# paultsw/wavenet-speech

Hardware: AMD Instinct MI355X
Metric: samples/sec fwd+bwd, 256-ch 30-block WaveNet @16k seq (higher is better)
Workload: dtype f32; 1 GPU; BASELINE.json configs[2]: WaveNet 256 ch, 30 blocks (3 x dilation 1..512), k=2, seq_len 16000, batch 16 per GPU, f32, full step (fwd+bwd+grad all-reduce+Adam); channels=256, blocks=30, seq_len=16000, batch_per_gpu=16, global_batch=16, parallelism=dp1, params=16037632, input=dense one-hot, init=reference

## Files before the change

wavenet_speech_amd/csrc/wn_gemm.hip:

```cpp
#include <cstdlib>
#include <type_traits>

#include "wn_kernels.h"
#include "wn_knobs.h"

namespace wn {

__device__ __forceinline__ int rowof(int r, int h) { return (r & 3) + 8 * (r >> 2) + 4 * h; }

__device__ __forceinline__ float sigmoid_f(float x) {
    const float e = __builtin_amdgcn_exp2f(-1.44269504088896341f * x);
    return __builtin_amdgcn_rcpf(1.0f + e);
}
__device__ __forceinline__ float tanh_f(float x) {
    const float ax = __builtin_fabsf(x);
    const float e = __builtin_amdgcn_exp2f(-2.88539008177792681f * ax);
    const float big = (1.0f - e) * __builtin_amdgcn_rcpf(1.0f + e);
    const float x2 = x * x;
    const float small = ax * (1.0f + x2 * (-0.333333333f + x2 * (0.133333333f + x2 * -0.0539682540f)));
    return __builtin_copysignf(ax < 0.125f ? small : big, x);
}

template <int NT> struct BVec;
template <> struct BVec<4> { typedef f32x4 reg_t; };
template <> struct BVec<2> { typedef float __attribute__((ext_vector_type(2))) reg_t; };

template <int MT, int NT, int EPI, int PFB, int WPS>
__global__ __launch_bounds__(64, WPS) void series_gemm_kernel(const GemmArgs a) {
    typedef typename BVec<NT>::reg_t breg_t;
    constexpr int COLS = 32 * NT;
    const int lane = threadIdx.x;
    const int n0 = lane & 31, h0 = lane >> 5;
#ifdef WN_STAMPS
    const unsigned long long st_t0 = __builtin_amdgcn_s_memtime(), st_r0 = __builtin_amdgcn_s_memrealtime();
    unsigned long long st_t1 = 0, st_t2 = 0;
#endif

    const int id = blockIdx.x;
    const int xcd = id & 7, local = id >> 3;
    const int slab_i = local % a.nslab;
    const int coltile = (local / a.nslab) * 8 + xcd;
    if (coltile >= a.ncol) return;
    const int b = coltile / a.tiles_per_row;
    const int t0 = (coltile - b * a.tiles_per_row) * COLS;
    const GemmSlab sl = a.slab[slab_i];
    const int ld = a.ld;

    f32x16 acc[MT][NT];
    const float* bias_p = (a.bias ? a.bias : a.wpacked) + sl.boff;
    const float bias_on = a.bias ? 1.0f : 0.0f;
#pragma unroll
    for (int m = 0; m < MT; ++m) {
#pragma unroll
        for (int r = 0; r < 16; ++r) {
            const float bv = bias_p[32 * m + rowof(r, h0)] * bias_on;
#pragma unroll
            for (int t = 0; t < NT; ++t) acc[m][t][r] = bv;
        }
    }

    int nkb = 0;
    for (int s = 0; s < sl.nseg; ++s) nkb += a.seg[s].nkb;

    constexpr unsigned kRsrcFlags = 0x00020000u;
    auto resource = [&](const float* base) {
        return __builtin_amdgcn_make_buffer_rsrc(const_cast<float*>(base), 0, 0xffffffffu, kRsrcFlags);
    };
    const __amdgpu_buffer_rsrc_t wrs = resource(a.wpacked + sl.woff);
    const unsigned a_off = lane * 16u;
    unsigned a_soff = 0;
    const long tilebase = (long)a.halo + t0;
    unsigned b_off[4];
#pragma unroll
    for (int q = 0; q < 4; ++q) b_off[q] = 4u * ((unsigned)(4 * h0 + q) * (unsigned)ld + (unsigned)(NT * n0));
    int seg = 0;
    int seg_left = a.seg[0].nkb;
    __amdgpu_buffer_rsrc_t brs = resource(a.seg[0].base + (long)b * a.seg[0].cp * ld);
    unsigned b_soff = 4u * (unsigned)(tilebase + a.seg[0].off);
    int b_left = nkb;
    const unsigned a_last = (unsigned)(nkb > 0 ? nkb - 1 : 0) * (MT * 1024u);

    f32x4 A[2][MT];
    breg_t B[4][4];
    auto loadA = [&](f32x4 (&dst)[MT]) {
#pragma unroll
        for (int m = 0; m < MT; ++m)
            dst[m] = __builtin_bit_cast(f32x4, __builtin_amdgcn_raw_buffer_load_b128(wrs, a_off + m * 1024u, a_soff, 0));
        a_soff = min(a_soff + MT * 1024u, a_last);
    };
    auto loadB = [&](breg_t (&dst)[4]) {
#pragma unroll
        for (int q = 0; q < 4; ++q) {
            if constexpr (NT == 4) dst[q] = __builtin_bit_cast(breg_t, __builtin_amdgcn_raw_buffer_load_b128(brs, b_off[q], b_soff, 0));
            else dst[q] = __builtin_bit_cast(breg_t, __builtin_amdgcn_raw_buffer_load_b64(brs, b_off[q], b_soff, 0));
        }
        const int more = min(b_left - 1, 1);
        b_left -= more;
        b_soff += (unsigned)more * (32u * (unsigned)ld);
        seg_left -= more;
        if (b_left > 1 - more && seg_left == 0) {
            ++seg;
            const GemmSeg ns = a.seg[seg];
            seg_left = ns.nkb;
            brs = resource(ns.base + (long)b * ns.cp * ld);
            b_soff = 4u * (unsigned)(tilebase + ns.off);
        }
    };
    auto compute = [&](const f32x4 (&fa)[MT], const breg_t (&fb)[4]) {
#pragma unroll
        for (int q = 0; q < 4; ++q)
#pragma unroll
            for (int m = 0; m < MT; ++m)
#pragma unroll
                for (int t = 0; t < NT; ++t)
                    acc[m][t] = __builtin_amdgcn_mfma_f32_32x32x2f32(fa[m][q], fb[q][t], acc[m][t], 0, 0, 0);
    };

    loadA(A[0]);
#pragma unroll
    for (int p = 0; p < PFB; ++p) loadB(B[p]);
#ifdef WN_STAMPS
    __builtin_amdgcn_sched_barrier(0);
    st_t1 = __builtin_amdgcn_s_memtime();
    __builtin_amdgcn_sched_barrier(0);
#endif
    int g0 = 0;
    for (; g0 + 4 <= nkb; g0 += 4) {
#pragma unroll
        for (int j = 0; j < 4; ++j) {
            loadA(A[(j + 1) & 1]);
            loadB(B[(j + PFB) & 3]);
            __builtin_amdgcn_sched_barrier(0);
            compute(A[j & 1], B[j & 3]);
            __builtin_amdgcn_sched_barrier(0);
        }
    }
#pragma unroll
    for (int j = 0; j < 3; ++j) {
        if (g0 + j < nkb) {
            loadA(A[(j + 1) & 1]);
            loadB(B[(j + PFB) & 3]);
            __builtin_amdgcn_sched_barrier(0);
            compute(A[j & 1], B[j & 3]);
            __builtin_amdgcn_sched_barrier(0);
        }
    }

#ifdef WN_STAMPS
    __builtin_amdgcn_sched_barrier(0);
    st_t2 = __builtin_amdgcn_s_memtime();
    __builtin_amdgcn_sched_barrier(0);
    struct StampOut {
        unsigned long long* p; unsigned long long t0, r0, t1, t2; int lane;
        __device__ ~StampOut() {
            __builtin_amdgcn_sched_barrier(0);
            const unsigned long long t_issued = __builtin_amdgcn_s_memtime();
            __builtin_amdgcn_sched_barrier(0);
            asm volatile("s_waitcnt vmcnt(0)" ::: "memory");
            if (p && lane == 0) {
                p[0] = t0; p[1] = t1; p[2] = t2; p[3] = __builtin_amdgcn_s_memtime();
                p[4] = r0; p[5] = __builtin_amdgcn_s_memrealtime();
                p[6] = __builtin_amdgcn_s_getreg(63492);
                p[7] = (unsigned long long)__builtin_amdgcn_s_getreg(63508) | ((t_issued - t2) << 32);
            }
        }
    } stamp_out{a.stamps ? a.stamps + 8ull * blockIdx.x : nullptr, st_t0, st_r0, st_t1, st_t2, lane};
#endif
    const int lane_e = (int)__builtin_amdgcn_mbcnt_hi(~0u, __builtin_amdgcn_mbcnt_lo(~0u, 0u));
    const int n = lane_e & 31, h = lane_e >> 5;
    const long colbase = tilebase + NT * n;
    const int c0 = t0 + NT * n;
    if (c0 >= a.L) return;
    auto clip = [&](breg_t v) {
#pragma unroll
        for (int t = 1; t < NT; ++t)
            if (c0 + t >= a.L) v[t] = 0.0f;
        return v;
    };
    [[maybe_unused]] auto both_forms = [&](int rows, auto&& body) {
        if (sl.row0 + 32 * MT <= rows && t0 + COLS <= a.L) body(std::true_type{});
        else body(std::false_type{});
    };

    if constexpr (EPI == EPI_LINEAR) {
        const GemmDst d = a.dst[sl.dst];
#pragma unroll
        for (int m = 0; m < MT; ++m) {
#pragma unroll
            for (int r = 0; r < 16; ++r) {
                const int row = sl.row0 + 32 * m + rowof(r, h);
                if (row < d.rows) {
                    float* p = d.base + ((long)b * d.cp + row) * ld + colbase;
                    breg_t v;
#pragma unroll
                    for (int t = 0; t < NT; ++t) v[t] = acc[m][t][r];
                    *reinterpret_cast<breg_t*>(p) = clip(v);
                }
            }
            __builtin_amdgcn_sched_barrier(0);
        }
    } else if constexpr (EPI == EPI_ACCUM) {
        const GemmDst d = a.dst[sl.dst];
        constexpr int RB = 8, BPT = 16 / RB, NBATCH = MT * BPT;
        float* const tile = d.base + (long)b * d.cp * ld + colbase;
        both_forms(d.rows, [&](auto full) {
            constexpr bool FULL = decltype(full)::value;
            breg_t old[2][RB];
            auto fetch = [&](int bi, breg_t (&dst)[RB]) {
                const int m = bi / BPT, r0 = (bi % BPT) * RB;
#pragma unroll
                for (int i = 0; i < RB; ++i) {
                    int row = sl.row0 + 32 * m + rowof(r0 + i, h);
                    if constexpr (!FULL) row = row < d.rows ? row : d.rows - 1;
                    dst[i] = *reinterpret_cast<const breg_t*>(tile + (long)row * ld);
                }
            };
            fetch(0, old[0]);
#pragma unroll
            for (int bi = 0; bi < NBATCH; ++bi) {
                if (bi + 1 < NBATCH) fetch(bi + 1, old[(bi + 1) & 1]);
                __builtin_amdgcn_sched_barrier(0);
                const int m = bi / BPT, r0 = (bi % BPT) * RB;
#pragma unroll
                for (int i = 0; i < RB; ++i) {
                    const int row = sl.row0 + 32 * m + rowof(r0 + i, h);
                    if (FULL || row < d.rows) {
                        breg_t v;
#pragma unroll
                        for (int t = 0; t < NT; ++t) v[t] = acc[m][t][r0 + i] + old[bi & 1][i][t];
                        *reinterpret_cast<breg_t*>(tile + (long)row * ld) = FULL ? v : clip(v);
                    }
                }
                __builtin_amdgcn_sched_barrier(0);
            }
        });
    } else if constexpr (EPI == EPI_GATE) {
#pragma unroll
        for (int i = 0; i < MT / 2; ++i) {
#pragma unroll
            for (int r = 0; r < 16; ++r) {
                const int ch = sl.row0 + 32 * i + rowof(r, h);
                if (ch < a.gate_rows) {
                    breg_t vs, vz;
#pragma unroll
                    for (int t = 0; t < NT; ++t) {
                        const float tt = tanh_f(acc[2 * i][t][r]);
                        const float ss = sigmoid_f(acc[2 * i + 1][t][r]);
                        vs[t] = ss;
                        vz[t] = tt * ss;
                    }
                    const long o = ((long)b * a.gate_cp + ch) * ld + colbase;
                    *reinterpret_cast<breg_t*>(a.z + o) = clip(vz);
                    if (a.sg) *reinterpret_cast<breg_t*>(a.sg + o) = clip(vs);
                }
            }
            __builtin_amdgcn_sched_barrier(0);
        }
    } else if constexpr (EPI == EPI_LEAKY) {
        const GemmDst d = a.dst[sl.dst];
        const float slope = a.slope;
#pragma unroll
        for (int m = 0; m < MT; ++m) {
#pragma unroll
            for (int r = 0; r < 16; ++r) {
                const int row = sl.row0 + 32 * m + rowof(r, h);
                if (row < d.rows) {
                    float* p = d.base + ((long)b * d.cp + row) * ld + colbase;
                    breg_t v;
#pragma unroll
                    for (int t = 0; t < NT; ++t) {
                        const float x = acc[m][t][r];
                        v[t] = x > 0.0f ? x : x * slope;
                    }
                    *reinterpret_cast<breg_t*>(p) = clip(v);
                }
            }
            __builtin_amdgcn_sched_barrier(0);
        }
    } else if constexpr (EPI == EPI_DMASK) {
        const GemmDst d = a.dst[sl.dst];
        const float slope = a.slope;
        constexpr int RB = 8, BPT = 16 / RB, NBATCH = MT * BPT;
        const long tile_off = (long)b * d.cp * ld + colbase;
        float* const tile = d.base + tile_off;
        const float* const mtile = a.mask + tile_off;
        both_forms(d.rows, [&](auto full) {
            constexpr bool FULL = decltype(full)::value;
            breg_t msk[2][RB];
            auto fetch = [&](int bi, breg_t (&dst)[RB]) {
                const int m = bi / BPT, r0 = (bi % BPT) * RB;
#pragma unroll
                for (int i = 0; i < RB; ++i) {
                    int row = sl.row0 + 32 * m + rowof(r0 + i, h);
                    if constexpr (!FULL) row = row < d.rows ? row : d.rows - 1;
                    dst[i] = *reinterpret_cast<const breg_t*>(mtile + (long)row * ld);
                }
            };
            fetch(0, msk[0]);
#pragma unroll
            for (int bi = 0; bi < NBATCH; ++bi) {
                if (bi + 1 < NBATCH) fetch(bi + 1, msk[(bi + 1) & 1]);
                __builtin_amdgcn_sched_barrier(0);
                const int m = bi / BPT, r0 = (bi % BPT) * RB;
#pragma unroll
                for (int i = 0; i < RB; ++i) {
                    const int row = sl.row0 + 32 * m + rowof(r0 + i, h);
                    if (FULL || row < d.rows) {
                        breg_t v;
#pragma unroll
                        for (int t = 0; t < NT; ++t) {
                            const float g = acc[m][t][r0 + i];
                            v[t] = msk[bi & 1][i][t] > 0.0f ? g : g * slope;
                        }
                        *reinterpret_cast<breg_t*>(tile + (long)row * ld) = FULL ? v : clip(v);
                    }
                }
                __builtin_amdgcn_sched_barrier(0);
            }
        });
    } else {
        constexpr int RB = (MT == 4) ? 8 : 4;
        constexpr int BPT = 16 / RB;
        constexpr int NBATCH = MT * BPT;
        both_forms(a.gate_rows, [&](auto full) {
            constexpr bool FULL = decltype(full)::value;
            breg_t vt[2][RB], vs[2][RB];
            const long plane = (long)b * a.gate_cp * ld;
            auto at = [&](auto* base, int ch) {
                if constexpr (FULL) return (decltype(base))((char*)(base + plane) + 4u * ((unsigned)ch * (unsigned)ld + (unsigned)colbase));
                else return base + ((long)b * a.gate_cp + ch) * ld + colbase;
            };
            auto fetch = [&](int bi, breg_t (&ft)[RB], breg_t (&fs)[RB]) {
                const int m = bi / BPT, r0 = (bi % BPT) * RB;
#pragma unroll
                for (int i = 0; i < RB; ++i) {
                    int ch = sl.row0 + 32 * m + rowof(r0 + i, h);
                    if constexpr (!FULL) ch = ch < a.gate_rows ? ch : a.gate_rows - 1;
                    ft[i] = *reinterpret_cast<const breg_t*>(at(a.z, ch));
                    fs[i] = *reinterpret_cast<const breg_t*>(at(a.sg, ch));
                }
            };
            fetch(0, vt[0], vs[0]);
#pragma unroll
            for (int bi = 0; bi < NBATCH; ++bi) {
                if (bi + 1 < NBATCH) fetch(bi + 1, vt[(bi + 1) & 1], vs[(bi + 1) & 1]);
                __builtin_amdgcn_sched_barrier(0);
                const int m = bi / BPT, r0 = (bi % BPT) * RB;
#pragma unroll
                for (int i = 0; i < RB; ++i) {
                    const int r = r0 + i;
                    const int ch = sl.row0 + 32 * m + rowof(r, h);
                    if (FULL || ch < a.gate_rows) {
                        const breg_t z_ = vt[bi & 1][i], sg_ = vs[bi & 1][i];
                        breg_t va, vg;
#pragma unroll
                        for (int t = 0; t < NT; ++t) {
                            const float dz = acc[m][t][r];
                            const float tt = sg_[t] > 0.0f ? z_[t] / sg_[t] : 0.0f;
                            va[t] = dz * (sg_[t] - z_[t] * tt);
                            vg[t] = dz * z_[t] * (1.0f - sg_[t]);
                        }
                        *reinterpret_cast<breg_t*>(at(a.da, ch)) = FULL ? va : clip(va);
                        *reinterpret_cast<breg_t*>(at(a.dg, ch)) = FULL ? vg : clip(vg);
                    }
                }
                __builtin_amdgcn_sched_barrier(0);
            }
        });
    }
}

#ifdef WN_STAMPS
static unsigned long long* g_stamp_buf = nullptr;
static int g_stamp_kc = -1;
int g_debug_kc = -1;
extern "C" void wn_debug_set_stamp_buffer(void* p) { g_stamp_buf = (unsigned long long*)p; }
extern "C" void wn_debug_set_stamp_class(int kc) { g_stamp_kc = kc; }
extern "C" unsigned wn_debug_last_grid = 0;
#endif

template <int MT, int NT, int EPI, int PFB, int WPS>
static hipError_t launch_one(GemmArgs a, hipStream_t st) {
#ifdef WN_STAMPS
    const bool stamp_this = g_stamp_buf && (g_stamp_kc < 0 || g_stamp_kc == g_debug_kc);
    a.stamps = stamp_this ? g_stamp_buf : nullptr;
#endif
    a.tiles_per_row = (a.L + 32 * NT - 1) / (32 * NT);
    a.ncol = a.B * a.tiles_per_row;
    const int ncol8 = (a.ncol + 7) / 8 * 8;
    const unsigned grid = (unsigned)(a.nslab * ncol8);
#ifdef WN_STAMPS
    if (stamp_this) wn_debug_last_grid = grid;
#endif
    hipLaunchKernelGGL((series_gemm_kernel<MT, NT, EPI, PFB, WPS>), dim3(grid), dim3(64), 0, st, a);
    return hipGetLastError();
}

template <int EPI>
static hipError_t launch_epi(int MT, const GemmArgs& a, hipStream_t st) {
    if (MT == 4) {
        if constexpr (kMeasureBuild) {
            if (measure_knob(Knob::WN_GEMM_VARIANT, 0) == 1) return launch_one<4, 4, EPI, 1, 1>(a, st);
        }
        return launch_one<4, 4, EPI, 3, 1>(a, st);
    }
    if (MT == 2) return launch_one<2, 4, EPI, 3, 2>(a, st);
    if constexpr (EPI != EPI_GATE) {
        if (MT == 1) return launch_one<1, 4, EPI, 3, 2>(a, st);
    }
    return hipErrorInvalidValue;
}

hipError_t launch_gemm(int MT, int epi, const GemmArgs& a, hipStream_t st) {
    if (a.nslab <= 0 || a.B <= 0 || a.L <= 0) return hipSuccess;
    switch (epi) {
        case EPI_LINEAR: return launch_epi<EPI_LINEAR>(MT, a, st);
        case EPI_GATE: return launch_epi<EPI_GATE>(MT, a, st);
        case EPI_DGATE: return launch_epi<EPI_DGATE>(MT, a, st);
        case EPI_ACCUM: return launch_epi<EPI_ACCUM>(MT, a, st);
        case EPI_LEAKY: return launch_epi<EPI_LEAKY>(MT, a, st);
        case EPI_DMASK: return launch_epi<EPI_DMASK>(MT, a, st);
    }
    return hipErrorInvalidValue;
}

}
```

Before: 101.5 samples/s.

## Add finishing-wave path that overlaps last k-blocks with epilogue for linear/leaky GEMMs

```diff
diff --git a/wavenet_speech_amd/csrc/wn_gemm.hip b/wavenet_speech_amd/csrc/wn_gemm.hip
--- a/wavenet_speech_amd/csrc/wn_gemm.hip
+++ b/wavenet_speech_amd/csrc/wn_gemm.hip
@@ -25,349 +25,37 @@
 template <> struct BVec<4> { typedef f32x4 reg_t; };
 template <> struct BVec<2> { typedef float __attribute__((ext_vector_type(2))) reg_t; };
 
+typedef unsigned u32x4 __attribute__((ext_vector_type(4)));
+
+#ifndef WN_FINISH_LINEAR
+#define WN_FINISH_LINEAR 2
+#endif
+constexpr int finish_blocks(int MT, int NT, int EPI, int PFB, int WPS) {
+    return (MT == 4 && NT == 4 && PFB == 3 && WPS == 1 && (EPI == EPI_LINEAR || EPI == EPI_LEAKY)) ? WN_FINISH_LINEAR : 0;
+}
+
+template <int MT, int NT, int EPI, int PFB, int WPS, int FT>
+__device__ __forceinline__ void series_gemm_finishing_wave(const GemmArgs& a) {
+#include "wn_gemm_wave.h"
+}
+
 template <int MT, int NT, int EPI, int PFB, int WPS>
 __global__ __launch_bounds__(64, WPS) void series_gemm_kernel(const GemmArgs a) {
-    typedef typename BVec<NT>::reg_t breg_t;
-    constexpr int COLS = 32 * NT;
-    const int lane = threadIdx.x;
-    const int n0 = lane & 31, h0 = lane >> 5;
-#ifdef WN_STAMPS
-    const unsigned long long st_t0 = __builtin_amdgcn_s_memtime(), st_r0 = __builtin_amdgcn_s_memrealtime();
-    unsigned long long st_t1 = 0, st_t2 = 0;
-#endif
-
-    const int id = blockIdx.x;
-    const int xcd = id & 7, local = id >> 3;
-    const int slab_i = local % a.nslab;
-    const int coltile = (local / a.nslab) * 8 + xcd;
-    if (coltile >= a.ncol) return;
-    const int b = coltile / a.tiles_per_row;
-    const int t0 = (coltile - b * a.tiles_per_row) * COLS;
-    const GemmSlab sl = a.slab[slab_i];
-    const int ld = a.ld;
-
-    f32x16 acc[MT][NT];
-    const float* bias_p = (a.bias ? a.bias : a.wpacked) + sl.boff;
-    const float bias_on = a.bias ? 1.0f : 0.0f;
-#pragma unroll
-    for (int m = 0; m < MT; ++m) {
-#pragma unroll
-        for (int r = 0; r < 16; ++r) {
-            const float bv = bias_p[32 * m + rowof(r, h0)] * bias_on;
-#pragma unroll
-            for (int t = 0; t < NT; ++t) acc[m][t][r] = bv;
+    if constexpr (finish_blocks(MT, NT, EPI, PFB, WPS) > 0) {
+        constexpr int FIN = finish_blocks(MT, NT, EPI, PFB, WPS);
+        const int local = blockIdx.x >> 3;
+        const int coltile = (local / a.nslab) * 8 + (blockIdx.x & 7);
+        const GemmSlab sl = a.slab[local % a.nslab];
+        int nkb = 0;
+        for (int s = 0; s < sl.nseg; ++s) nkb += a.seg[s].nkb;
+        const int t0 = (coltile % a.tiles_per_row) * 32 * NT;
+        if (coltile < a.ncol && nkb >= FIN && sl.row0 + 32 * MT <= a.dst[sl.dst].rows && t0 + 32 * NT <= a.L) {
+            series_gemm_finishing_wave<MT, NT, EPI, PFB, WPS, FIN>(a);
+            return;
         }
     }
-
-    int nkb = 0;
-    for (int s = 0; s < sl.nseg; ++s) nkb += a.seg[s].nkb;
-
-    constexpr unsigned kRsrcFlags = 0x00020000u;
-    auto resource = [&](const float* base) {
-        return __builtin_amdgcn_make_buffer_rsrc(const_cast<float*>(base), 0, 0xffffffffu, kRsrcFlags);
-    };
-    const __amdgpu_buffer_rsrc_t wrs = resource(a.wpacked + sl.woff);
-    const unsigned a_off = lane * 16u;
-    unsigned a_soff = 0;
-    const long tilebase = (long)a.halo + t0;
-    unsigned b_off[4];
-#pragma unroll
-    for (int q = 0; q < 4; ++q) b_off[q] = 4u * ((unsigned)(4 * h0 + q) * (unsigned)ld + (unsigned)(NT * n0));
-    int seg = 0;
-    int seg_left = a.seg[0].nkb;
-    __amdgpu_buffer_rsrc_t brs = resource(a.seg[0].base + (long)b * a.seg[0].cp * ld);
-    unsigned b_soff = 4u * (unsigned)(tilebase + a.seg[0].off);
-    int b_left = nkb;
-    const unsigned a_last = (unsigned)(nkb > 0 ? nkb - 1 : 0) * (MT * 1024u);
-
-    f32x4 A[2][MT];
-    breg_t B[4][4];
-    auto loadA = [&](f32x4 (&dst)[MT]) {
-#pragma unroll
-        for (int m = 0; m < MT; ++m)
-            dst[m] = __builtin_bit_cast(f32x4, __builtin_amdgcn_raw_buffer_load_b128(wrs, a_off + m * 1024u, a_soff, 0));
-        a_soff = min(a_soff + MT * 1024u, a_last);
-    };
-    auto loadB = [&](breg_t (&dst)[4]) {
-#pragma unroll
-        for (int q = 0; q < 4; ++q) {
-            if constexpr (NT == 4) dst[q] = __builtin_bit_cast(breg_t, __builtin_amdgcn_raw_buffer_load_b128(brs, b_off[q], b_soff, 0));
-            else dst[q] = __builtin_bit_cast(breg_t, __builtin_amdgcn_raw_buffer_load_b64(brs, b_off[q], b_soff, 0));
-        }
-        const int more = min(b_left - 1, 1);
-        b_left -= more;
-        b_soff += (unsigned)more * (32u * (unsigned)ld);
-        seg_left -= more;
-        if (b_left > 1 - more && seg_left == 0) {
-            ++seg;
-            const GemmSeg ns = a.seg[seg];
-            seg_left = ns.nkb;
-            brs = resource(ns.base + (long)b * ns.cp * ld);
-            b_soff = 4u * (unsigned)(tilebase + ns.off);
-        }
-    };
-    auto compute = [&](const f32x4 (&fa)[MT], const breg_t (&fb)[4]) {
-#pragma unroll
-        for (int q = 0; q < 4; ++q)
-#pragma unroll
-            for (int m = 0; m < MT; ++m)
-#pragma unroll
-                for (int t = 0; t < NT; ++t)
-                    acc[m][t] = __builtin_amdgcn_mfma_f32_32x32x2f32(fa[m][q], fb[q][t], acc[m][t], 0, 0, 0);
-    };
-
-    loadA(A[0]);
-#pragma unroll
-    for (int p = 0; p < PFB; ++p) loadB(B[p]);
-#ifdef WN_STAMPS
-    __builtin_amdgcn_sched_barrier(0);
-    st_t1 = __builtin_amdgcn_s_memtime();
-    __builtin_amdgcn_sched_barrier(0);
-#endif
-    int g0 = 0;
-    for (; g0 + 4 <= nkb; g0 += 4) {
-#pragma unroll
-        for (int j = 0; j < 4; ++j) {
-            loadA(A[(j + 1) & 1]);
-            loadB(B[(j + PFB) & 3]);
-            __builtin_amdgcn_sched_barrier(0);
-            compute(A[j & 1], B[j & 3]);
-            __builtin_amdgcn_sched_barrier(0);
-        }
-    }
-#pragma unroll
-    for (int j = 0; j < 3; ++j) {
-        if (g0 + j < nkb) {
-            loadA(A[(j + 1) & 1]);
-            loadB(B[(j + PFB) & 3]);
-            __builtin_amdgcn_sched_barrier(0);
-            compute(A[j & 1], B[j & 3]);
-            __builtin_amdgcn_sched_barrier(0);
-        }
-    }
-
-#ifdef WN_STAMPS
-    __builtin_amdgcn_sched_barrier(0);
-    st_t2 = __builtin_amdgcn_s_memtime();
-    __builtin_amdgcn_sched_barrier(0);
-    struct StampOut {
-        unsigned long long* p; unsigned long long t0, r0, t1, t2; int lane;
-        __device__ ~StampOut() {
-            __builtin_amdgcn_sched_barrier(0);
-            const unsigned long long t_issued = __builtin_amdgcn_s_memtime();
-            __builtin_amdgcn_sched_barrier(0);
-            asm volatile("s_waitcnt vmcnt(0)" ::: "memory");
-            if (p && lane == 0) {
-                p[0] = t0; p[1] = t1; p[2] = t2; p[3] = __builtin_amdgcn_s_memtime();
-                p[4] = r0; p[5] = __builtin_amdgcn_s_memrealtime();
-                p[6] = __builtin_amdgcn_s_getreg(63492);
-                p[7] = (unsigned long long)__builtin_amdgcn_s_getreg(63508) | ((t_issued - t2) << 32);
-            }
-        }
-    } stamp_out{a.stamps ? a.stamps + 8ull * blockIdx.x : nullptr, st_t0, st_r0, st_t1, st_t2, lane};
-#endif
-    const int lane_e = (int)__builtin_amdgcn_mbcnt_hi(~0u, __builtin_amdgcn_mbcnt_lo(~0u, 0u));
-    const int n = lane_e & 31, h = lane_e >> 5;
-    const long colbase = tilebase + NT * n;
-    const int c0 = t0 + NT * n;
-    if (c0 >= a.L) return;
-    auto clip = [&](breg_t v) {
-#pragma unroll
-        for (int t = 1; t < NT; ++t)
-            if (c0 + t >= a.L) v[t] = 0.0f;
-        return v;
-    };
-    [[maybe_unused]] auto both_forms = [&](int rows, auto&& body) {
-        if (sl.row0 + 32 * MT <= rows && t0 + COLS <= a.L) body(std::true_type{});
-        else body(std::false_type{});
-    };
-
-    if constexpr (EPI == EPI_LINEAR) {
-        const GemmDst d = a.dst[sl.dst];
-#pragma unroll
-        for (int m = 0; m < MT; ++m) {
-#pragma unroll
-            for (int r = 0; r < 16; ++r) {
-                const int row = sl.row0 + 32 * m + rowof(r, h);
-                if (row < d.rows) {
-                    float* p = d.base + ((long)b * d.cp + row) * ld + colbase;
-                    breg_t v;
-#pragma unroll
-                    for (int t = 0; t < NT; ++t) v[t] = acc[m][t][r];
-                    *reinterpret_cast<breg_t*>(p) = clip(v);
-                }
-            }
-            __builtin_amdgcn_sched_barrier(0);
-        }
-    } else if constexpr (EPI == EPI_ACCUM) {
-        const GemmDst d = a.dst[sl.dst];
-        constexpr int RB = 8, BPT = 16 / RB, NBATCH = MT * BPT;
-        float* const tile = d.base + (long)b * d.cp * ld + colbase;
-        both_forms(d.rows, [&](auto full) {
-            constexpr bool FULL = decltype(full)::value;
-            breg_t old[2][RB];
-            auto fetch = [&](int bi, breg_t (&dst)[RB]) {
-                const int m = bi / BPT, r0 = (bi % BPT) * RB;
-#pragma unroll
-                for (int i = 0; i < RB; ++i) {
-                    int row = sl.row0 + 32 * m + rowof(r0 + i, h);
-                    if constexpr (!FULL) row = row < d.rows ? row : d.rows - 1;
-                    dst[i] = *reinterpret_cast<const breg_t*>(tile + (long)row * ld);
-                }
-            };
-            fetch(0, old[0]);
-#pragma unroll
-            for (int bi = 0; bi < NBATCH; ++bi) {
-                if (bi + 1 < NBATCH) fetch(bi + 1, old[(bi + 1) & 1]);
-                __builtin_amdgcn_sched_barrier(0);
-                const int m = bi / BPT, r0 = (bi % BPT) * RB;
-#pragma unroll
-                for (int i = 0; i < RB; ++i) {
-                    const int row = sl.row0 + 32 * m + rowof(r0 + i, h);
-                    if (FULL || row < d.rows) {
-                        breg_t v;
-#pragma unroll
-                        for (int t = 0; t < NT; ++t) v[t] = acc[m][t][r0 + i] + old[bi & 1][i][t];
-                        *reinterpret_cast<breg_t*>(tile + (long)row * ld) = FULL ? v : clip(v);
-                    }
-                }
-                __builtin_amdgcn_sched_barrier(0);
-            }
-        });
-    } else if constexpr (EPI == EPI_GATE) {
-#pragma unroll
-        for (int i = 0; i < MT / 2; ++i) {
-#pragma unroll
-            for (int r = 0; r < 16; ++r) {
-                const int ch = sl.row0 + 32 * i + rowof(r, h);
-                if (ch < a.gate_rows) {
-                    breg_t vs, vz;
-#pragma unroll
-                    for (int t = 0; t < NT; ++t) {
-                        const float tt = tanh_f(acc[2 * i][t][r]);
-                        const float ss = sigmoid_f(acc[2 * i + 1][t][r]);
-                        vs[t] = ss;
-                        vz[t] = tt * ss;
-                    }
-                    const long o = ((long)b * a.gate_cp + ch) * ld + colbase;
-                    *reinterpret_cast<breg_t*>(a.z + o) = clip(vz);
-                    if (a.sg) *reinterpret_cast<breg_t*>(a.sg + o) = clip(vs);
-                }
-            }
-            __builtin_amdgcn_sched_barrier(0);
-        }
-    } else if constexpr (EPI == EPI_LEAKY) {
-        const GemmDst d = a.dst[sl.dst];
-        const float slope = a.slope;
-#pragma unroll
-        for (int m = 0; m < MT; ++m) {
-#pragma unroll
-            for (int r = 0; r < 16; ++r) {
-                const int row = sl.row0 + 32 * m + rowof(r, h);
-                if (row < d.rows) {
-                    float* p = d.base + ((long)b * d.cp + row) * ld + colbase;
-                    breg_t v;
-#pragma unroll
-                    for (int t = 0; t < NT; ++t) {
-                        const float x = acc[m][t][r];
-                        v[t] = x > 0.0f ? x : x * slope;
-                    }
-                    *reinterpret_cast<breg_t*>(p) = clip(v);
-                }
-            }
-            __builtin_amdgcn_sched_barrier(0);
-        }
-    } else if constexpr (EPI == EPI_DMASK) {
-        const GemmDst d = a.dst[sl.dst];
-        const float slope = a.slope;
-        constexpr int RB = 8, BPT = 16 / RB, NBATCH = MT * BPT;
-        const long tile_off = (long)b * d.cp * ld + colbase;
-        float* const tile = d.base + tile_off;
-        const float* const mtile = a.mask + tile_off;
-        both_forms(d.rows, [&](auto full) {
-            constexpr bool FULL = decltype(full)::value;
-            breg_t msk[2][RB];
-            auto fetch = [&](int bi, breg_t (&dst)[RB]) {
-                const int m = bi / BPT, r0 = (bi % BPT) * RB;
-#pragma unroll
-                for (int i = 0; i < RB; ++i) {
-                    int row = sl.row0 + 32 * m + rowof(r0 + i, h);
-                    if constexpr (!FULL) row = row < d.rows ? row : d.rows - 1;
-                    dst[i] = *reinterpret_cast<const breg_t*>(mtile + (long)row * ld);
-                }
-            };
-            fetch(0, msk[0]);
-#pragma unroll
-            for (int bi = 0; bi < NBATCH; ++bi) {
-                if (bi + 1 < NBATCH) fetch(bi + 1, msk[(bi + 1) & 1]);
-                __builtin_amdgcn_sched_barrier(0);
-                const int m = bi / BPT, r0 = (bi % BPT) * RB;
-#pragma unroll
-                for (int i = 0; i < RB; ++i) {
-                    const int row = sl.row0 + 32 * m + rowof(r0 + i, h);
-                    if (FULL || row < d.rows) {
-                        breg_t v;
-#pragma unroll
-                        for (int t = 0; t < NT; ++t) {
-                            const float g = acc[m][t][r0 + i];
-                            v[t] = msk[bi & 1][i][t] > 0.0f ? g : g * slope;
-                        }
-                        *reinterpret_cast<breg_t*>(tile + (long)row * ld) = FULL ? v : clip(v);
-                    }
-                }
-                __builtin_amdgcn_sched_barrier(0);
-            }
-        });
-    } else {
-        constexpr int RB = (MT == 4) ? 8 : 4;
-        constexpr int BPT = 16 / RB;
-        constexpr int NBATCH = MT * BPT;
-        both_forms(a.gate_rows, [&](auto full) {
-            constexpr bool FULL = decltype(full)::value;
-            breg_t vt[2][RB], vs[2][RB];
-            const long plane = (long)b * a.gate_cp * ld;
-            auto at = [&](auto* base, int ch) {
-                if constexpr (FULL) return (decltype(base))((char*)(base + plane) + 4u * ((unsigned)ch * (unsigned)ld + (unsigned)colbase));
-                else return base + ((long)b * a.gate_cp + ch) * ld + colbase;
-            };
-            auto fetch = [&](int bi, breg_t (&ft)[RB], breg_t (&fs)[RB]) {
-                const int m = bi / BPT, r0 = (bi % BPT) * RB;
-#pragma unroll
-                for (int i = 0; i < RB; ++i) {
-                    int ch = sl.row0 + 32 * m + rowof(r0 + i, h);
-                    if constexpr (!FULL) ch = ch < a.gate_rows ? ch : a.gate_rows - 1;
-                    ft[i] = *reinterpret_cast<const breg_t*>(at(a.z, ch));
-                    fs[i] = *reinterpret_cast<const breg_t*>(at(a.sg, ch));
-                }
-            };
-            fetch(0, vt[0], vs[0]);
-#pragma unroll
-            for (int bi = 0; bi < NBATCH; ++bi) {
-                if (bi + 1 < NBATCH) fetch(bi + 1, vt[(bi + 1) & 1], vs[(bi + 1) & 1]);
-                __builtin_amdgcn_sched_barrier(0);
-                const int m = bi / BPT, r0 = (bi % BPT) * RB;
-#pragma unroll
-                for (int i = 0; i < RB; ++i) {
-                    const int r = r0 + i;
-                    const int ch = sl.row0 + 32 * m + rowof(r, h);
-                    if (FULL || ch < a.gate_rows) {
-                        const breg_t z_ = vt[bi & 1][i], sg_ = vs[bi & 1][i];
-                        breg_t va, vg;
-#pragma unroll
-                        for (int t = 0; t < NT; ++t) {
-                            const float dz = acc[m][t][r];
-                            const float tt = sg_[t] > 0.0f ? z_[t] / sg_[t] : 0.0f;
-                            va[t] = dz * (sg_[t] - z_[t] * tt);
-                            vg[t] = dz * z_[t] * (1.0f - sg_[t]);
-                        }
-                        *reinterpret_cast<breg_t*>(at(a.da, ch)) = FULL ? va : clip(va);
-                        *reinterpret_cast<breg_t*>(at(a.dg, ch)) = FULL ? vg : clip(vg);
-                    }
-                }
-                __builtin_amdgcn_sched_barrier(0);
-            }
-        });
-    }
+    constexpr int FT = 0;
+#include "wn_gemm_wave.h"
 }
 
 #ifdef WN_STAMPS
diff --git a/wavenet_speech_amd/csrc/wn_gemm_wave.h b/wavenet_speech_amd/csrc/wn_gemm_wave.h
--- /dev/null
+++ b/wavenet_speech_amd/csrc/wn_gemm_wave.h
@@ -0,0 +1,407 @@
+    typedef typename BVec<NT>::reg_t breg_t;
+    constexpr int COLS = 32 * NT;
+    const int lane = threadIdx.x;
+    const int n0 = lane & 31, h0 = lane >> 5;
+#ifdef WN_STAMPS
+    const unsigned long long st_t0 = __builtin_amdgcn_s_memtime(), st_r0 = __builtin_amdgcn_s_memrealtime();
+    unsigned long long st_t1 = 0;
+#endif
+
+    const int id = blockIdx.x;
+    const int xcd = id & 7, local = id >> 3;
+    const int slab_i = local % a.nslab;
+    const int coltile = (local / a.nslab) * 8 + xcd;
+    if (coltile >= a.ncol) return;
+    const int b = coltile / a.tiles_per_row;
+    const int t0 = (coltile - b * a.tiles_per_row) * COLS;
+    const GemmSlab sl = a.slab[slab_i];
+    const int ld = a.ld;
+
+    f32x16 acc[MT][NT];
+    const float* bias_p = (a.bias ? a.bias : a.wpacked) + sl.boff;
+    const float bias_on = a.bias ? 1.0f : 0.0f;
+#pragma unroll
+    for (int m = 0; m < MT; ++m) {
+#pragma unroll
+        for (int r = 0; r < 16; ++r) {
+            const float bv = bias_p[32 * m + rowof(r, h0)] * bias_on;
+#pragma unroll
+            for (int t = 0; t < NT; ++t) acc[m][t][r] = bv;
+        }
+    }
+
+    int nkb = 0;
+    for (int s = 0; s < sl.nseg; ++s) nkb += a.seg[s].nkb;
+
+    constexpr unsigned kRsrcFlags = 0x00020000u;
+    auto resource = [&](const float* base) {
+        return __builtin_amdgcn_make_buffer_rsrc(const_cast<float*>(base), 0, 0xffffffffu, kRsrcFlags);
+    };
+    const __amdgpu_buffer_rsrc_t wrs = resource(a.wpacked + sl.woff);
+    const unsigned a_off = lane * 16u;
+    unsigned a_soff = 0;
+    const long tilebase = (long)a.halo + t0;
+    unsigned b_off[4];
+#pragma unroll
+    for (int q = 0; q < 4; ++q) b_off[q] = 4u * ((unsigned)(4 * h0 + q) * (unsigned)ld + (unsigned)(NT * n0));
+    int seg = 0;
+    int seg_left = a.seg[0].nkb;
+    __amdgpu_buffer_rsrc_t brs = resource(a.seg[0].base + (long)b * a.seg[0].cp * ld);
+    unsigned b_soff = 4u * (unsigned)(tilebase + a.seg[0].off);
+    int b_left = nkb;
+    const unsigned a_last = (unsigned)(nkb > 0 ? nkb - 1 : 0) * (MT * 1024u);
+
+    f32x4 A[2][MT];
+    breg_t B[4][4];
+    auto loadA = [&](f32x4 (&dst)[MT]) {
+#pragma unroll
+        for (int m = 0; m < MT; ++m)
+            dst[m] = __builtin_bit_cast(f32x4, __builtin_amdgcn_raw_buffer_load_b128(wrs, a_off + m * 1024u, a_soff, 0));
+        a_soff = min(a_soff + MT * 1024u, a_last);
+    };
+    auto loadB = [&](breg_t (&dst)[4]) {
+#pragma unroll
+        for (int q = 0; q < 4; ++q) {
+            if constexpr (NT == 4) dst[q] = __builtin_bit_cast(breg_t, __builtin_amdgcn_raw_buffer_load_b128(brs, b_off[q], b_soff, 0));
+            else dst[q] = __builtin_bit_cast(breg_t, __builtin_amdgcn_raw_buffer_load_b64(brs, b_off[q], b_soff, 0));
+        }
+        const int more = min(b_left - 1, 1);
+        b_left -= more;
+        b_soff += (unsigned)more * (32u * (unsigned)ld);
+        seg_left -= more;
+        if (b_left > 1 - more && seg_left == 0) {
+            ++seg;
+            const GemmSeg ns = a.seg[seg];
+            seg_left = ns.nkb;
+            brs = resource(ns.base + (long)b * ns.cp * ld);
+            b_soff = 4u * (unsigned)(tilebase + ns.off);
+        }
+    };
+    auto compute = [&](const f32x4 (&fa)[MT], const breg_t (&fb)[4]) {
+#pragma unroll
+        for (int q = 0; q < 4; ++q)
+#pragma unroll
+            for (int m = 0; m < MT; ++m)
+#pragma unroll
+                for (int t = 0; t < NT; ++t)
+                    acc[m][t] = __builtin_amdgcn_mfma_f32_32x32x2f32(fa[m][q], fb[q][t], acc[m][t], 0, 0, 0);
+    };
+
+    const int n_main = nkb - FT;
+
+    loadA(A[0]);
+#pragma unroll
+    for (int p = 0; p < PFB; ++p) loadB(B[p]);
+#ifdef WN_STAMPS
+    __builtin_amdgcn_sched_barrier(0);
+    st_t1 = __builtin_amdgcn_s_memtime();
+    __builtin_amdgcn_sched_barrier(0);
+    struct StampOut {
+        unsigned long long* p; unsigned long long t0, r0, t1, t2; int lane;
+        __device__ ~StampOut() {
+            __builtin_amdgcn_sched_barrier(0);
+            const unsigned long long t_issued = __builtin_amdgcn_s_memtime();
+            __builtin_amdgcn_sched_barrier(0);
+            asm volatile("s_waitcnt vmcnt(0)" ::: "memory");
+            if (p && lane == 0) {
+                p[0] = t0; p[1] = t1; p[2] = t2; p[3] = __builtin_amdgcn_s_memtime();
+                p[4] = r0; p[5] = __builtin_amdgcn_s_memrealtime();
+                p[6] = __builtin_amdgcn_s_getreg(63492);
+                p[7] = (unsigned long long)__builtin_amdgcn_s_getreg(63508) | ((t_issued - t2) << 32);
+            }
+        }
+    } stamp_out{a.stamps ? a.stamps + 8ull * blockIdx.x : nullptr, st_t0, st_r0, st_t1, 0, lane};
+#endif
+    int g0 = 0;
+    for (; g0 + 4 <= n_main; g0 += 4) {
+#pragma unroll
+        for (int j = 0; j < 4; ++j) {
+            loadA(A[(j + 1) & 1]);
+            loadB(B[(j + PFB) & 3]);
+            __builtin_amdgcn_sched_barrier(0);
+            compute(A[j & 1], B[j & 3]);
+            __builtin_amdgcn_sched_barrier(0);
+        }
+    }
+#pragma unroll
+    for (int j = 0; j < 3; ++j) {
+        if (g0 + j < n_main) {
+            loadA(A[(j + 1) & 1]);
+            loadB(B[(j + PFB) & 3]);
+            __builtin_amdgcn_sched_barrier(0);
+            compute(A[j & 1], B[j & 3]);
+            __builtin_amdgcn_sched_barrier(0);
+        }
+    }
+
+    if constexpr (FT > 0) {
+        static_assert(FT == 2 && PFB == 3 && MT == 4 && NT == 4, "the finishing phase takes its operands from the rings as they stand");
+        const GemmDst d = a.dst[sl.dst];
+        [[maybe_unused]] const float slope = a.slope;
+        const int lane_f = (int)__builtin_amdgcn_mbcnt_hi(~0u, __builtin_amdgcn_mbcnt_lo(~0u, 0u));
+        const __amdgpu_buffer_rsrc_t drs = resource(d.base + (long)b * d.cp * ld);
+        const unsigned v_off = 4u * ((unsigned)(4 * (lane_f >> 5)) * (unsigned)ld + (unsigned)tilebase + (unsigned)(NT * (lane_f & 31)));
+        constexpr int G = 4 * FT;
+        constexpr int UNITS = 16 * MT;
+        auto unit = [&](int u) {
+            const int m = u / 16, r = u % 16;
+            f32x4 v;
+#pragma unroll
+            for (int t = 0; t < NT; ++t) {
+                float x;
+                asm volatile("v_accvgpr_read_b32 %0, %1" : "=v"(x) : "a"(acc[m][t][r]));
+                v[t] = (EPI == EPI_LEAKY) ? (x > 0.0f ? x : x * slope) : x;
+            }
+            const unsigned s_off = 4u * (unsigned)(sl.row0 + 32 * m + (r & 3) + 8 * (r >> 2)) * (unsigned)ld;
+            __builtin_amdgcn_raw_buffer_store_b128(__builtin_bit_cast(u32x4, v), drs, v_off, s_off, 0);
+        };
+        f32x4 FA[2][MT];
+        breg_t FB[2][4];
+        auto take = [&](auto ring) {
+            constexpr int R = decltype(ring)::value;
+#pragma unroll
+            for (int m = 0; m < MT; ++m) FA[0][m] = A[R & 1][m];
+#pragma unroll
+            for (int q = 0; q < 4; ++q) { FB[0][q] = B[R & 3][q]; FB[1][q] = B[(R + 1) & 3][q]; }
+        };
+        switch (n_main & 3) {
+            case 0: take(std::integral_constant<int, 0>{}); break;
+            case 1: take(std::integral_constant<int, 1>{}); break;
+            case 2: take(std::integral_constant<int, 2>{}); break;
+            default: take(std::integral_constant<int, 3>{}); break;
+        }
+        loadA(FA[1]);
+        __builtin_amdgcn_sched_barrier(0);
+#pragma unroll
+        for (int m = 0; m < MT; ++m)
+#pragma unroll
+            for (int kb = 0; kb < FT; ++kb)
+#pragma unroll
+                for (int q = 0; q < 4; ++q) {
+                    const int u = (m * FT + kb) * 4 + q - G - 1;
+                    if (u >= 0) unit(u);
+                    __builtin_amdgcn_sched_barrier(0);
+#pragma unroll
+                    for (int t = 0; t < NT; ++t)
+                        acc[m][t] = __builtin_amdgcn_mfma_f32_32x32x2f32(FA[kb][m][q], FB[kb][q][t], acc[m][t], 0, 0, 0);
+                    __builtin_amdgcn_sched_barrier(0);
+                }
+#ifdef WN_STAMPS
+        stamp_out.t2 = __builtin_amdgcn_s_memtime();
+        __builtin_amdgcn_sched_barrier(0);
+#endif
+#pragma unroll
+        for (int u = MT * G - G - 1; u < UNITS; ++u) {
+            if (u == UNITS - 16) asm volatile("s_nop 15\n\ts_nop 3");
+            unit(u);
+        }
+        return;
+    }
+
+#ifdef WN_STAMPS
+    __builtin_amdgcn_sched_barrier(0);
+    stamp_out.t2 = __builtin_amdgcn_s_memtime();
+    __builtin_amdgcn_sched_barrier(0);
+#endif
+    const int lane_e = (int)__builtin_amdgcn_mbcnt_hi(~0u, __builtin_amdgcn_mbcnt_lo(~0u, 0u));
+    const int n = lane_e & 31, h = lane_e >> 5;
+    const long colbase = tilebase + NT * n;
+    const int c0 = t0 + NT * n;
+    if (c0 >= a.L) return;
+    auto clip = [&](breg_t v) {
+#pragma unroll
+        for (int t = 1; t < NT; ++t)
+            if (c0 + t >= a.L) v[t] = 0.0f;
+        return v;
+    };
+    [[maybe_unused]] auto both_forms = [&](int rows, auto&& body) {
+        if (sl.row0 + 32 * MT <= rows && t0 + COLS <= a.L) body(std::true_type{});
+        else body(std::false_type{});
+    };
+
+    if constexpr (EPI == EPI_LINEAR) {
+        const GemmDst d = a.dst[sl.dst];
+#pragma unroll
+        for (int m = 0; m < MT; ++m) {
+#pragma unroll
+            for (int r = 0; r < 16; ++r) {
+                const int row = sl.row0 + 32 * m + rowof(r, h);
+                if (row < d.rows) {
+                    float* p = d.base + ((long)b * d.cp + row) * ld + colbase;
+                    breg_t v;
+#pragma unroll
+                    for (int t = 0; t < NT; ++t) v[t] = acc[m][t][r];
+                    *reinterpret_cast<breg_t*>(p) = clip(v);
+                }
+            }
+            __builtin_amdgcn_sched_barrier(0);
+        }
+    } else if constexpr (EPI == EPI_ACCUM) {
+        const GemmDst d = a.dst[sl.dst];
+        constexpr int RB = 8, BPT = 16 / RB, NBATCH = MT * BPT;
+        float* const tile = d.base + (long)b * d.cp * ld + colbase;
+        both_forms(d.rows, [&](auto full) {
+            constexpr bool FULL = decltype(full)::value;
+            breg_t old[2][RB];
+            auto fetch = [&](int bi, breg_t (&dst)[RB]) {
+                const int m = bi / BPT, r0 = (bi % BPT) * RB;
+#pragma unroll
+                for (int i = 0; i < RB; ++i) {
+                    int row = sl.row0 + 32 * m + rowof(r0 + i, h);
+                    if constexpr (!FULL) row = row < d.rows ? row : d.rows - 1;
+                    dst[i] = *reinterpret_cast<const breg_t*>(tile + (long)row * ld);
+                }
+            };
+            fetch(0, old[0]);
+#pragma unroll
+            for (int bi = 0; bi < NBATCH; ++bi) {
+                if (bi + 1 < NBATCH) fetch(bi + 1, old[(bi + 1) & 1]);
+                __builtin_amdgcn_sched_barrier(0);
+                const int m = bi / BPT, r0 = (bi % BPT) * RB;
+#pragma unroll
+                for (int i = 0; i < RB; ++i) {
+                    const int row = sl.row0 + 32 * m + rowof(r0 + i, h);
+                    if (FULL || row < d.rows) {
+                        breg_t v;
+#pragma unroll
+                        for (int t = 0; t < NT; ++t) v[t] = acc[m][t][r0 + i] + old[bi & 1][i][t];
+                        *reinterpret_cast<breg_t*>(tile + (long)row * ld) = FULL ? v : clip(v);
+                    }
+                }
+                __builtin_amdgcn_sched_barrier(0);
+            }
+        });
+    } else if constexpr (EPI == EPI_GATE) {
+#pragma unroll
+        for (int i = 0; i < MT / 2; ++i) {
+#pragma unroll
+            for (int r = 0; r < 16; ++r) {
+                const int ch = sl.row0 + 32 * i + rowof(r, h);
+                if (ch < a.gate_rows) {
+                    breg_t vs, vz;
+#pragma unroll
+                    for (int t = 0; t < NT; ++t) {
+                        const float tt = tanh_f(acc[2 * i][t][r]);
+                        const float ss = sigmoid_f(acc[2 * i + 1][t][r]);
+                        vs[t] = ss;
+                        vz[t] = tt * ss;
+                    }
+                    const long o = ((long)b * a.gate_cp + ch) * ld + colbase;
+                    *reinterpret_cast<breg_t*>(a.z + o) = clip(vz);
+                    if (a.sg) *reinterpret_cast<breg_t*>(a.sg + o) = clip(vs);
+                }
+            }
+            __builtin_amdgcn_sched_barrier(0);
+        }
+    } else if constexpr (EPI == EPI_LEAKY) {
+        const GemmDst d = a.dst[sl.dst];
+        const float slope = a.slope;
+#pragma unroll
+        for (int m = 0; m < MT; ++m) {
+#pragma unroll
+            for (int r = 0; r < 16; ++r) {
+                const int row = sl.row0 + 32 * m + rowof(r, h);
+                if (row < d.rows) {
+                    float* p = d.base + ((long)b * d.cp + row) * ld + colbase;
+                    breg_t v;
+#pragma unroll
+                    for (int t = 0; t < NT; ++t) {
+                        const float x = acc[m][t][r];
+                        v[t] = x > 0.0f ? x : x * slope;
+                    }
+                    *reinterpret_cast<breg_t*>(p) = clip(v);
+                }
+            }
+            __builtin_amdgcn_sched_barrier(0);
+        }
+    } else if constexpr (EPI == EPI_DMASK) {
+        const GemmDst d = a.dst[sl.dst];
+        const float slope = a.slope;
+        constexpr int RB = 8, BPT = 16 / RB, NBATCH = MT * BPT;
+        const long tile_off = (long)b * d.cp * ld + colbase;
+        float* const tile = d.base + tile_off;
+        const float* const mtile = a.mask + tile_off;
+        both_forms(d.rows, [&](auto full) {
+            constexpr bool FULL = decltype(full)::value;
+            breg_t msk[2][RB];
+            auto fetch = [&](int bi, breg_t (&dst)[RB]) {
+                const int m = bi / BPT, r0 = (bi % BPT) * RB;
+#pragma unroll
+                for (int i = 0; i < RB; ++i) {
+                    int row = sl.row0 + 32 * m + rowof(r0 + i, h);
+                    if constexpr (!FULL) row = row < d.rows ? row : d.rows - 1;
+                    dst[i] = *reinterpret_cast<const breg_t*>(mtile + (long)row * ld);
+                }
+            };
+            fetch(0, msk[0]);
+#pragma unroll
+            for (int bi = 0; bi < NBATCH; ++bi) {
+                if (bi + 1 < NBATCH) fetch(bi + 1, msk[(bi + 1) & 1]);
+                __builtin_amdgcn_sched_barrier(0);
+                const int m = bi / BPT, r0 = (bi % BPT) * RB;
+#pragma unroll
+                for (int i = 0; i < RB; ++i) {
+                    const int row = sl.row0 + 32 * m + rowof(r0 + i, h);
+                    if (FULL || row < d.rows) {
+                        breg_t v;
+#pragma unroll
+                        for (int t = 0; t < NT; ++t) {
+                            const float g = acc[m][t][r0 + i];
+                            v[t] = msk[bi & 1][i][t] > 0.0f ? g : g * slope;
+                        }
+                        *reinterpret_cast<breg_t*>(tile + (long)row * ld) = FULL ? v : clip(v);
+                    }
+                }
+                __builtin_amdgcn_sched_barrier(0);
+            }
+        });
+    } else {
+        constexpr int RB = (MT == 4) ? 8 : 4;
+        constexpr int BPT = 16 / RB;
+        constexpr int NBATCH = MT * BPT;
+        both_forms(a.gate_rows, [&](auto full) {
+            constexpr bool FULL = decltype(full)::value;
+            breg_t vt[2][RB], vs[2][RB];
+            const long plane = (long)b * a.gate_cp * ld;
+            auto at = [&](auto* base, int ch) {
+                if constexpr (FULL) return (decltype(base))((char*)(base + plane) + 4u * ((unsigned)ch * (unsigned)ld + (unsigned)colbase));
+                else return base + ((long)b * a.gate_cp + ch) * ld + colbase;
+            };
+            auto fetch = [&](int bi, breg_t (&ft)[RB], breg_t (&fs)[RB]) {
+                const int m = bi / BPT, r0 = (bi % BPT) * RB;
+#pragma unroll
+                for (int i = 0; i < RB; ++i) {
+                    int ch = sl.row0 + 32 * m + rowof(r0 + i, h);
+                    if constexpr (!FULL) ch = ch < a.gate_rows ? ch : a.gate_rows - 1;
+                    ft[i] = *reinterpret_cast<const breg_t*>(at(a.z, ch));
+                    fs[i] = *reinterpret_cast<const breg_t*>(at(a.sg, ch));
+                }
+            };
+            fetch(0, vt[0], vs[0]);
+#pragma unroll
+            for (int bi = 0; bi < NBATCH; ++bi) {
+                if (bi + 1 < NBATCH) fetch(bi + 1, vt[(bi + 1) & 1], vs[(bi + 1) & 1]);
+                __builtin_amdgcn_sched_barrier(0);
+                const int m = bi / BPT, r0 = (bi % BPT) * RB;
+#pragma unroll
+                for (int i = 0; i < RB; ++i) {
+                    const int r = r0 + i;
+                    const int ch = sl.row0 + 32 * m + rowof(r, h);
+                    if (FULL || ch < a.gate_rows) {
+                        const breg_t z_ = vt[bi & 1][i], sg_ = vs[bi & 1][i];
+                        breg_t va, vg;
+#pragma unroll
+                        for (int t = 0; t < NT; ++t) {
+                            const float dz = acc[m][t][r];
+                            const float tt = sg_[t] > 0.0f ? z_[t] / sg_[t] : 0.0f;
+                            va[t] = dz * (sg_[t] - z_[t] * tt);
+                            vg[t] = dz * z_[t] * (1.0f - sg_[t]);
+                        }
+                        *reinterpret_cast<breg_t*>(at(a.da, ch)) = FULL ? va : clip(va);
+                        *reinterpret_cast<breg_t*>(at(a.dg, ch)) = FULL ? vg : clip(vg);
+                    }
+                }
+                __builtin_amdgcn_sched_barrier(0);
+            }
+        });
+    }
```

After: 101.8 samples/s, median of 6. No clear change (+0.3%).
